# stelleg/caster-dta

Hardware: AMD Instinct MI355X
Metric: graph-pairs/sec (Davis-shaped protein+drug), encoders fwd+bwd (higher is better)
Workload: dtype f32; 1 GPU; davis_b64; pairs_per_gpu=64, residues_per_gpu=19200, protein_edges_per_gpu=57484, atoms_per_gpu=2560, drug_edges_per_gpu=7986, encoder=CASTER-DTA(2,2), pass=fwdbwd, activation_storage=fp32, scope=encoders, torch_compile=False, tunable_gemms=False, two_lane_head=False, train_mode=True, csr_build_in_step=True, hip_graph=True, kernels=mfma

## Files before the change

caster-dta_amd/csrc/gvp_quad.h:

```cpp
#pragma once
#include <hip/hip_runtime.h>

#include "gvp_math.h"

namespace gq {

typedef float f4 __attribute__((ext_vector_type(4)));

constexpr int P1 = 0, P2 = 1;
constexpr int ceil4(int x) { return (x + 3) / 4; }

struct bf16s {};
template <typename ST> struct Io;
template <> struct Io<float> {
  static constexpr bool BF = false;
  static __device__ __forceinline__ f4 ld4(const float* p, int64_t i) { return *reinterpret_cast<const f4*>(p + i); }
  static __device__ __forceinline__ float ld(const float* p, int64_t i) { return p[i]; }
  static __device__ __forceinline__ void st4(float* p, int64_t i, f4 v) { *reinterpret_cast<f4*>(p + i) = v; }
  static __device__ __forceinline__ void st(float* p, int64_t i, float v) { p[i] = v; }
  static __device__ __forceinline__ float rt(float v) { return v; }
  static __device__ __forceinline__ f4 rt4(f4 v) { return v; }
};
struct f32_gvpdef {};
struct f32_linear {};
template <> struct Io<bf16s> {
  static constexpr bool BF = true;
  static __device__ __forceinline__ float widen(uint32_t hi16) { return __uint_as_float(hi16); }
  static __device__ __forceinline__ uint16_t narrow(float v) { return __builtin_bit_cast(uint16_t, (__bf16)v); }
  static __device__ __forceinline__ f4 ld4(const float* p, int64_t i) {
    const uint2 u = *reinterpret_cast<const uint2*>(reinterpret_cast<const uint16_t*>(p) + i);
    return f4{widen(u.x << 16), widen(u.x & 0xffff0000u), widen(u.y << 16), widen(u.y & 0xffff0000u)};
  }
  static __device__ __forceinline__ float ld(const float* p, int64_t i) {
    return widen((uint32_t)reinterpret_cast<const uint16_t*>(p)[i] << 16);
  }
  static __device__ __forceinline__ void st4(float* p, int64_t i, f4 v) {
    uint2 u;
    u.x = (uint32_t)narrow(v[0]) | ((uint32_t)narrow(v[1]) << 16);
    u.y = (uint32_t)narrow(v[2]) | ((uint32_t)narrow(v[3]) << 16);
    *reinterpret_cast<uint2*>(reinterpret_cast<uint16_t*>(p) + i) = u;
  }
  static __device__ __forceinline__ void st(float* p, int64_t i, float v) { reinterpret_cast<uint16_t*>(p)[i] = narrow(v); }
  static __device__ __forceinline__ float rt(float v) { return widen((uint32_t)narrow(v) << 16); }
  static __device__ __forceinline__ f4 rt4(f4 v) { return f4{rt(v[0]), rt(v[1]), rt(v[2]), rt(v[3])}; }
};

template <> struct Io<f32_gvpdef> : Io<float> {};
template <> struct Io<f32_linear> : Io<float> {};

template <int KIND, int BASE, int WIDTH>
struct Seg {
  static_assert(KIND == P2 || WIDTH % 16 == 0, "P1 segments are whole 16-channel tiles");
  static constexpr int steps = KIND == P1 ? WIDTH / 4 : ceil4(WIDTH);
  static __host__ __device__ int col(int s, int g) {
    if (KIND == P1) return BASE + 16 * (s >> 2) + 4 * g + (s & 3);
    const int c = 4 * s + g;
    return c < WIDTH ? BASE + c : -1;
  }
};

template <int STEPS>
struct SegNone {
  static constexpr int steps = STEPS;
  static __host__ __device__ int col(int, int) { return -1; }
};

template <class... S>
struct Segs {
  static constexpr int steps = (S::steps + ... + 0);
  static __host__ __device__ int col(int s, int g) {
    int res = -1, s0 = 0;
    ((res = (s >= s0 && s < s0 + S::steps) ? S::col(s - s0, g) : res, s0 += S::steps), ...);
    return res;
  }
};

template <int NSTEPS>
__host__ __device__ inline void frag_decode(int idx, int& mt, int& s, int& lane) {
  constexpr int REGION = NSTEPS * 64, FULL = NSTEPS / 4;
  mt = idx / REGION;
  const int u = idx - mt * REGION;
  if (u < FULL * 256) { s = 4 * (u >> 8) + (u & 3); lane = (u & 255) >> 2; }
  else { const int v = u - FULL * 256; s = 4 * FULL + (v >> 6); lane = v & 63; }
}
// ... 917 lines not shown
          for (int j = 0; j < TN; ++j) outer_items<1, 1, BF>(AV[j], BH[j], w.vv);
        }
      }
    }
    if constexpr (PACK_V) {
#pragma unroll
      for (int p = 0; p < 3; ++p) {
        f4 A2[TN][1], B2[TN][1];
#pragma unroll
        for (int j = 0; j < TN; ++j) {
          float a2[VOR + HR], b2[HR + VSTEPS];
#pragma unroll
          for (int r = 0; r < VOR; ++r) a2[r] = gr[j].dvp[p][r];
#pragma unroll
          for (int r = 0; r < HR; ++r) a2[VOR + r] = gr[j].dvh[p][r];
#pragma unroll
          for (int r = 0; r < HR; ++r) b2[r] = c[j].vh[p][r];
#pragma unroll
          for (int s_ = 0; s_ < VSTEPS; ++s_) b2[HR + s_] = bv[j][p][s_];
          transpose_slots<VOR + HR>(a2, A2[j], lane, tscr + j * TSCR_FLOATS);
          transpose_slots<HR + VSTEPS>(b2, B2[j], lane, tscr + j * TSCR_FLOATS);
        }
#pragma unroll
        for (int j = 0; j < TN; ++j) outer_items<1, 1, BF>(A2[j], B2[j], w.vv);
      }
    } else {
#pragma unroll
      for (int p = 0; p < 3; ++p) {
        f4 AH[TN][1], BI[TN][1];
#pragma unroll
        for (int j = 0; j < TN; ++j) {
          float ah[HR], bin[VSTEPS];
#pragma unroll
          for (int r = 0; r < HR; ++r) ah[r] = gr[j].dvh[p][r];
#pragma unroll
          for (int s = 0; s < VSTEPS; ++s) bin[s] = bv[j][p][s];
          transpose_slots<HR>(ah, AH[j], lane, tscr + j * TSCR_FLOATS);
          transpose_slots<VSTEPS>(bin, BI[j], lane, tscr + j * TSCR_FLOATS);
        }
#pragma unroll
        for (int j = 0; j < TN; ++j) outer_items<1, 1, BF>(AH[j], BI[j], w.vh_);
      }
    }
  }
  template <class Acc>
  static __device__ __forceinline__ void wacc_flush(const WAcc& w, float* gblk, int lane) {
    const int i = lane & 15, g = lane >> 4;
    const bool first = false;
    flush_slots<Acc, Segs<Seg<P1, 0, SO>>, WsCols, OT, NBT>(gblk + A::ws(NT), first, K, w.ws, lane);
#pragma unroll
    for (int t = 0; t < OT; ++t) {
      float tot[4];
      float* q[4];
      bool on[4];
#pragma unroll
      for (int r = 0; r < 4; ++r) {
        tot[r] = row_total(w.bs[t][r]);
        q[r] = gblk + A::bs(NT) + 16 * t + 4 * g + r;
        on[r] = i == 15;
      }
      add_where<Acc, 4>(q, on, tot);
    }
    if (VO > 0) {
      flush_slots<Acc, Segs<Seg<P2, 0, (VO > 0 ? VO : 1)>>, Segs<Seg<P1, 0, SO>>, 1, OT>(gblk + A::wsv(NT), first, SO, w.wsv, lane);
      float tot[VOR];
      float* q[VOR];
      bool on[VOR];
#pragma unroll
      for (int r = 0; r < VOR; ++r) {
        tot[r] = row_total(w.bsv[r]);
        q[r] = gblk + A::bsv(NT) + 4 * r + g;
        on[r] = i == 15 && 4 * r + g < VO;
      }
      add_where<Acc, VOR>(q, on, tot);
      if constexpr (!PACK_V)
        flush_slots<Acc, Segs<Seg<P2, 0, (VO > 0 ? VO : 1)>>, Segs<Seg<P2, 0, H>>, 1, 1>(gblk + A::wv(NT), first, H, w.vv, lane);
    }
    if constexpr (PACK_V) {
      flush_slots<Acc, Segs<Seg<P2, 0, (VO > 0 ? VO : 1)>, SegNone<HR>>, Segs<Seg<P2, 0, H>, SegNone<VSTEPS>>, 1, 1>(
          gblk + A::wv(NT), first, H, w.vv, lane);
      flush_slots<Acc, Segs<SegNone<VOR>, Seg<P2, 0, H>>, Segs<SegNone<HR>, VSegs>, 1, 1>(gblk, first, VI, w.vv, lane);
    } else {
      flush_slots<Acc, Segs<Seg<P2, 0, H>>, VSegs, 1, 1>(gblk, first, VI, w.vh_, lane);
    }
  }
};

template <int S, int NV>
__device__ __forceinline__ void ln_quad(const float* ln, int lane, f4 (&s)[S / 16], float (&v)[3][ceil4(NV)]) {
  const int g = lane >> 4;
  float sum = 0.f;
#pragma unroll
  for (int t = 0; t < S / 16; ++t) sum += s[t][0] + s[t][1] + s[t][2] + s[t][3];
  const float mean = quad_sum(sum) * (1.0f / S);
  float var = 0.f;
#pragma unroll
  for (int t = 0; t < S / 16; ++t)
#pragma unroll
    for (int r = 0; r < 4; ++r) { const float d = s[t][r] - mean; var = fmaf(d, d, var); }
  const float rstd = gvp::f_rsqrt(quad_sum(var) * (1.0f / S) + gvp::kLnEps);
#pragma unroll
  for (int t = 0; t < S / 16; ++t) {
    const f4 ga = *reinterpret_cast<const f4*>(ln + 16 * t + 4 * g);
    const f4 be = *reinterpret_cast<const f4*>(ln + S + 16 * t + 4 * g);
#pragma unroll
    for (int r = 0; r < 4; ++r) s[t][r] = fmaf((s[t][r] - mean) * rstd, ga[r], be[r]);
  }
  float n2 = 0.f;
#pragma unroll
  for (int r = 0; r < ceil4(NV); ++r)
    if (4 * r + g < NV)
      n2 += gvp::f_max(v[0][r] * v[0][r] + v[1][r] * v[1][r] + v[2][r] * v[2][r], gvp::kNormEps);
  const float rvn = gvp::f_rsqrt(quad_sum(n2) * (1.0f / NV));
#pragma unroll
  for (int p = 0; p < 3; ++p)
#pragma unroll
    for (int r = 0; r < ceil4(NV); ++r) v[p][r] *= rvn;
}

template <int S, int NV>
__device__ __forceinline__ void ln_quad_bwd(const float* ln, int lane, const f4 (&x)[S / 16],
                                            const float (&v)[3][ceil4(NV)], f4 (&ds)[S / 16],
                                            float (&dv)[3][ceil4(NV)], f4 (&dgamma)[S / 16], f4 (&dbeta)[S / 16]) {
  const int g = lane >> 4;
  float sum = 0.f;
#pragma unroll
  for (int t = 0; t < S / 16; ++t) sum += x[t][0] + x[t][1] + x[t][2] + x[t][3];
  const float mean = quad_sum(sum) * (1.0f / S);
  float var = 0.f;
#pragma unroll
  for (int t = 0; t < S / 16; ++t)
#pragma unroll
    for (int r = 0; r < 4; ++r) { const float d = x[t][r] - mean; var = fmaf(d, d, var); }
  const float rstd = gvp::f_rsqrt(quad_sum(var) * (1.0f / S) + gvp::kLnEps);
  f4 xh[S / 16], dxh[S / 16];
  float m1 = 0.f, m2 = 0.f;
#pragma unroll
  for (int t = 0; t < S / 16; ++t) {
    const f4 ga = *reinterpret_cast<const f4*>(ln + 16 * t + 4 * g);
#pragma unroll
    for (int r = 0; r < 4; ++r) {
      xh[t][r] = (x[t][r] - mean) * rstd;
      dgamma[t][r] = ds[t][r] * xh[t][r];
      dbeta[t][r] = ds[t][r];
      dxh[t][r] = ds[t][r] * ga[r];
      m1 += dxh[t][r];
      m2 = fmaf(dxh[t][r], xh[t][r], m2);
    }
  }
  m1 = quad_sum(m1) * (1.0f / S);
  m2 = quad_sum(m2) * (1.0f / S);
#pragma unroll
  for (int t = 0; t < S / 16; ++t)
#pragma unroll
    for (int r = 0; r < 4; ++r) ds[t][r] = rstd * (dxh[t][r] - m1 - xh[t][r] * m2);
  float n2s = 0.f, dot = 0.f;
  bool free_[ceil4(NV)];
#pragma unroll
  for (int r = 0; r < ceil4(NV); ++r) {
    free_[r] = false;
    if (4 * r + g < NV) {
      const float n2 = v[0][r] * v[0][r] + v[1][r] * v[1][r] + v[2][r] * v[2][r];
      free_[r] = n2 > gvp::kNormEps;
      n2s += gvp::f_max(n2, gvp::kNormEps);
      dot += dv[0][r] * v[0][r] + dv[1][r] * v[1][r] + dv[2][r] * v[2][r];
    }
// ... 65 lines not shown
```

caster-dta_amd/csrc/gvp_quad_bwd_kernels.hip:

```cpp
#include <hip/hip_runtime.h>
#include <stdint.h>
#include <stdlib.h>

#include <type_traits>

#include "gvp_internal.h"
#include "gvp_quad.h"

using namespace gq;

#ifdef CGVP_STAMPS
__device__ unsigned long long* g_stamp_buf_bwd = nullptr;
extern "C" int cgvp_debug_set_stamp_buffer_bwd(unsigned long long* buf) {
  return (int)hipMemcpyToSymbol(HIP_SYMBOL(g_stamp_buf_bwd), &buf, sizeof(buf));
}
#endif

namespace {

constexpr int WAVE = 64;
constexpr int TILE = 16;

#ifdef CGVP_STAMPS
#define STAMP(slot)                                                                          \
// ... 28 lines not shown
__device__ __forceinline__ int opaque_lane(int lane) {
  asm volatile("" : "+v"(lane));
  return lane;
}

template <int BLK>
__device__ __forceinline__ void zero_block(float* gblk, int lane) {
  static_assert(BLK % 4 == 0, "blocks are whole float4s");
  for (int k = lane; k < BLK / 4; k += WAVE) reinterpret_cast<f4*>(gblk)[k] = f4{0.f, 0.f, 0.f, 0.f};
}
template <int BLK, int PW, int WPB_ = 8>
__device__ __forceinline__ void write_slab_row(float* slab, const float* blocks, int row = blockIdx.x) {
  __syncthreads();
  float* out = slab + (size_t)row * BLK;
  for (int k = threadIdx.x; k < BLK; k += WAVE * WPB_) {
    float t = 0.f;
#pragma unroll
    for (int ww = 0; ww < WPB_; ++ww) t += blocks[ww * PW + k];
    out[k] = t;
  }
}

template <int NFLOATS, int NTHR>
__device__ __forceinline__ void stage_slice(float* lds, const float* __restrict__ src, int tid) {
  static_assert(NFLOATS % 4 == 0, "image slices are whole float4s");
  constexpr int NF4 = NFLOATS / 4, IT = (NF4 + NTHR - 1) / NTHR;
  const f4* s = reinterpret_cast<const f4*>(src);
  f4* d = reinterpret_cast<f4*>(lds);
  f4 v[IT];
#pragma unroll
  for (int k = 0; k < IT; ++k) { const int idx = tid + k * NTHR; if (idx < NF4) v[k] = s[idx]; }
#pragma unroll
  for (int k = 0; k < IT; ++k) { const int idx = tid + k * NTHR; if (idx < NF4) d[idx] = v[k]; }
}

constexpr int cmax(int a, int b) { return a > b ? a : b; }
template <bool ONE> using AccFor = typename std::conditional<ONE, AccStoreOnce, AccPriv>::type;
constexpr int pad4(int x) { return (x + 3) / 4 * 4; }

template <class Acc, int S>
__device__ __forceinline__ void ln_param_grads(float* blk, bool first, int lane, bool active,
                                               const f4 (&dgamma)[S / 16], const f4 (&dbeta)[S / 16]) {
  const int i = lane & 15, g = lane >> 4;
#pragma unroll
  for (int t = 0; t < S / 16; ++t) {
    float tot[8];
    float* q[8];
    bool on[8];
#pragma unroll
    for (int r = 0; r < 4; ++r) {
      tot[r] = row_total(active ? dgamma[t][r] : 0.f);
      tot[4 + r] = row_total(active ? dbeta[t][r] : 0.f);
      q[r] = blk + 16 * t + 4 * g + r;
      q[4 + r] = blk + S + 16 * t + 4 * g + r;
      on[r] = on[4 + r] = i == 15;
    }
    add_where<Acc, 8>(q, on, tot);
  }
}

constexpr int NB_LN0 = 0, NB_LN1 = 2 * NS, NB_FF0 = 4 * NS, NB_FF1 = NB_FF0 + LFf0::size(0),
              NODE_BLK = NB_FF1 + LFf1::size(0);
constexpr int HB_LN = 0, HB_GVP = 2 * NS, HEAD_BLK = HB_GVP + LHead::size(0);
constexpr int NODE_GB = pad4(NODE_BLK), HEAD_GB = pad4(HEAD_BLK);

constexpr int MROW = NS + NV;
__device__ __forceinline__ void node_dropout(const float* mask, const gvp::RngArgs& rng, int which, int64_t n, int g,
                                             f4& ms, float& mv) {
  if (mask) {
    ms = *reinterpret_cast<const f4*>(mask + n * MROW + 4 * g);
    mv = mask[n * MROW + NS + g];
  } else if (rng.seed) {
    const unsigned long long seed = rng.seed[0], off = rng.seed[1];
    float fs[4];
    gvp::dropout_row20(seed, off, rng.stream + which, n, g, rng.p, fs, mv);
    ms = f4{fs[0], fs[1], fs[2], fs[3]};
  }
}
struct NodeBArgs {
  const float* img_node; const float* imgT_node;
  const float* h; const float* dh; const float* mask0; const float* mask1; gvp::RngArgs rng;
  const float* g_up0; const float* g_up1; const float* g_up2;
  int64_t N; float* g_dh; float* g_h; float* zero_rows; float* slab;
};
constexpr int node_bwd_lds_floats() { return BW_TPB + Image<0, 0>::ND_SIZE + Image<0, 0>::TN_SIZE + BW_WPB * (NODE_GB + TSCR_FLOATS); }
static_assert(node_bwd_lds_floats() * 4 <= 160 * 1024, "node backward LDS plan exceeds the CU");

template <typename ST, bool ONE = false>
__device__ __forceinline__ void node_bwd_body(const NodeBArgs& a, float* lds) {
  typedef Image<0, 0> IM;
  typedef AccFor<ONE> Acc;
  float* f_node = lds + BW_TPB;
  float* t_node = f_node + IM::ND_SIZE;
  float* blocks = t_node + IM::TN_SIZE;
  const int lane0 = threadIdx.x & 63, w = threadIdx.x >> 6;
  float* gblk = blocks + w * NODE_GB;
  float* tscr = blocks + BW_WPB * NODE_GB + w * TSCR_FLOATS;
  stage_slice<IM::ND_SIZE, BW_TPB>(f_node, a.img_node, threadIdx.x);
  stage_slice<IM::TN_SIZE, BW_TPB>(t_node, a.imgT_node, threadIdx.x);
  zero_block<NODE_GB>(gblk, lane0);
  STAMP(0);
  __syncthreads();
  STAMP(1);

  const f4 zero = {0.f, 0.f, 0.f, 0.f};
  const int zt[1] = {0};
  const bool first = false;
  const int64_t ntiles = (a.N + TILE - 1) / TILE;
  for (int64_t tile = (int64_t)w * gridDim.x + blockIdx.x; tile < ntiles; tile += (int64_t)gridDim.x * BW_WPB) {
    const int lane = opaque_lane(lane0), i = lane & 15, g = lane >> 4;
    const int64_t n = tile * TILE + i;
    const bool active = n < a.N;
    f4 x0[1] = {zero};
    float xv0[3][1] = {{0.f}, {0.f}, {0.f}};
    f4 m0s = {1.f, 1.f, 1.f, 1.f}, m1s = {1.f, 1.f, 1.f, 1.f};
    float m0v = 1.f, m1v = 1.f;
    f4 gs[1] = {zero};
    float gv[3][1] = {{0.f}, {0.f}, {0.f}};
    if (active) {
      const int64_t hr = n * ROW;
      node_dropout(a.mask0, a.rng, 0, n, g, m0s, m0v);
      node_dropout(a.mask1, a.rng, 1, n, g, m1s, m1v);
      x0[0] = Io<ST>::ld4(a.h, hr + 4 * g) + Io<ST>::ld4(a.dh, hr + 4 * g) * m0s;
#pragma unroll
      for (int p = 0; p < 3; ++p) xv0[p][0] = Io<ST>::ld(a.h, hr + NS + 3 * g + p) + Io<ST>::ld(a.dh, hr + NS + 3 * g + p) * m0v;
      const float* ups[3] = {a.g_up0, a.g_up1, a.g_up2};
#pragma unroll
      for (int u = 0; u < 3; ++u)
        if (ups[u]) {
          const float* r_ = ups[u] + n * ROW;
          gs[0] += *reinterpret_cast<const f4*>(r_ + 4 * g);
#pragma unroll
          for (int p = 0; p < 3; ++p) gv[p][0] += r_[NS + 3 * g + p];
        }
    }
    f4 y[1] = {x0[0]};
    float yv[3][1] = {{xv0[0][0]}, {xv0[1][0]}, {xv0[2][0]}};
    ln_quad<NS, NV>(f_node + IM::ND_LN0, lane, y, yv);
    f4 hs[1][4], s2[1][1];
    float hv[1][3][2], v2[1][3][1];
    float bs0[1][4], bv0[1][3][1], bs1[1][16], bv1[1][3][2];
    typename Ff0<ST>::Cache c0[1];
    typename Ff1<ST>::Cache c1[1];
#pragma unroll
    for (int r = 0; r < 4; ++r) bs0[0][r] = y[0][r];
#pragma unroll
    for (int p = 0; p < 3; ++p) bv0[0][p][0] = yv[p][0];
    Ff0<ST>::template forward<1, Io<ST>::BF>(f_node + IM::ND_FF0, lane, zt, bs0, bv0, hs, hv, c0);
#pragma unroll
    for (int t = 0; t < 4; ++t)
#pragma unroll
      for (int r = 0; r < 4; ++r) bs1[0][4 * t + r] = hs[0][t][r];
#pragma unroll
    for (int p = 0; p < 3; ++p) { bv1[0][p][0] = hv[0][p][0]; bv1[0][p][1] = hv[0][p][1]; }
    Ff1<ST>::template forward<1, Io<ST>::BF>(f_node + IM::ND_FF1, lane, zt, bs1, bv1, s2, v2, c1);
    f4 z[1] = {y[0] + s2[0][0] * m1s};
    float zv[3][1];
#pragma unroll
    for (int p = 0; p < 3; ++p) zv[p][0] = yv[p][0] + v2[0][p][0] * m1v;

    STAMP(2);
    STAMP(3);
    {
      f4 dga[1], dbe[1];
      ln_quad_bwd<NS, NV>(f_node + IM::ND_LN1, lane, z, zv, gs, gv, dga, dbe);
      ln_param_grads<Acc, NS>(gblk + NB_LN1, first, lane, active, dga, dbe);
    }
    float d_hs[16], d_hv[3][2];
    {
      f4 d_so[1] = {gs[0] * m1s};
      float d_vo[3][1] = {{gv[0][0] * m1v}, {gv[1][0] * m1v}, {gv[2][0] * m1v}};
      typename Ff1<ST>::Grads gr1;
      STAMP(4);
      Ff1<ST>::template backward<Io<ST>::BF>(t_node + IM::TN_FF1, lane, c1[0], d_so, d_vo, d_hs, d_hv, gr1);
      STAMP(5);
      Ff1<ST>::template weight_grads<Acc, Io<ST>::BF>(gblk + NB_FF1, first, lane, 0, active, bs1[0], bv1[0], c1[0], gr1, tscr);
    }
    {
      f4 d_so[4];
#pragma unroll
      for (int t = 0; t < 4; ++t) d_so[t] = f4{d_hs[4 * t], d_hs[4 * t + 1], d_hs[4 * t + 2], d_hs[4 * t + 3]};
      float d_ys[4], d_yv[3][1];
      typename Ff0<ST>::Grads gr0;
      STAMP(6);
      Ff0<ST>::template backward<Io<ST>::BF>(t_node + IM::TN_FF0, lane, c0[0], d_so, d_hv, d_ys, d_yv, gr0);
      STAMP(7);
      Ff0<ST>::template weight_grads<Acc, Io<ST>::BF>(gblk + NB_FF0, first, lane, 0, active, bs0[0], bv0[0], c0[0], gr0, tscr);
#pragma unroll
      for (int r = 0; r < 4; ++r) gs[0][r] += d_ys[r];
#pragma unroll
      for (int p = 0; p < 3; ++p) gv[p][0] += d_yv[p][0];
    }
    STAMP(8);
    {
      f4 dga[1], dbe[1];
      ln_quad_bwd<NS, NV>(f_node + IM::ND_LN0, lane, x0, xv0, gs, gv, dga, dbe);
      ln_param_grads<Acc, NS>(gblk + NB_LN0, first, lane, active, dga, dbe);
    }
    if (active) {
      if (a.g_h) {
        float* row = a.g_h + n * ROW;
        *reinterpret_cast<f4*>(row + 4 * g) = gs[0];
#pragma unroll
        for (int p = 0; p < 3; ++p) row[NS + 3 * g + p] = gv[p][0];
      }
      float* row = a.g_dh + n * ROW;
      *reinterpret_cast<f4*>(row + 4 * g) = gs[0] * m0s;
#pragma unroll
      for (int p = 0; p < 3; ++p) row[NS + 3 * g + p] = gv[p][0] * m0v;
      if (a.zero_rows) {
        float* z = a.zero_rows + n * ROW;
        *reinterpret_cast<f4*>(z + 4 * g) = zero;
#pragma unroll
        for (int p = 0; p < 3; ++p) z[NS + 3 * g + p] = 0.f;
      }
    }
  }
  STAMP(9);
  write_slab_row<NODE_GB, NODE_GB>(a.slab, blocks);
  STAMP(10);
}
template <typename ST, bool ONE = false>
__global__ __launch_bounds__(BW_TPB, 2) void node_bwd_kernel(NodeBArgs a) {
  WALL_STAMP(0);
  extern __shared__ __attribute__((aligned(16))) float lds[];
  node_bwd_body<ST, ONE>(a, lds);
}

struct HeadBArgs {
  const float* img_head; const float* imgT_head; const float* h_out; const float* g_out;
  int64_t N; float* g_h_out; float* slab;
};
constexpr int head_bwd_lds_floats() { return BW_TPB + Image<0, 0>::HD_SIZE + Image<0, 0>::TH_SIZE + BW_WPB * (HEAD_GB + TSCR_FLOATS); }

template <typename ST, bool ONE = false>
__device__ __forceinline__ void head_bwd_body(const HeadBArgs& a, float* lds) {
  typedef Image<0, 0> IM;
  typedef AccFor<ONE> Acc;
  float* f_head = lds + BW_TPB;
  float* t_head = f_head + IM::HD_SIZE;
  float* blocks = t_head + IM::TH_SIZE;
  const int lane = threadIdx.x & 63, w = threadIdx.x >> 6;
  float* gblk = blocks + w * HEAD_GB;
  float* tscr = blocks + BW_WPB * HEAD_GB + w * TSCR_FLOATS;
  stage_slice<IM::HD_SIZE, BW_TPB>(f_head, a.img_head, threadIdx.x);
  stage_slice<IM::TH_SIZE, BW_TPB>(t_head, a.imgT_head, threadIdx.x);
  zero_block<HEAD_GB>(gblk, lane);
  __syncthreads();

  const int i = lane & 15, g = lane >> 4;
  const f4 zero = {0.f, 0.f, 0.f, 0.f};
  const int zt[1] = {0};
  const bool first = false;
  const int64_t ntiles = (a.N + TILE - 1) / TILE;
  for (int64_t tile = (int64_t)w * gridDim.x + blockIdx.x; tile < ntiles; tile += (int64_t)gridDim.x * BW_WPB) {
    const int64_t n = tile * TILE + i;
    const bool active = n < a.N;
    f4 o1[1] = {zero};
    float ov1[3][1] = {{0.f}, {0.f}, {0.f}};
    f4 d_o[4] = {zero, zero, zero, zero};
    if (active) {
      const int64_t hr = n * ROW;
      o1[0] = Io<ST>::ld4(a.h_out, hr + 4 * g);
#pragma unroll
      for (int p = 0; p < 3; ++p) ov1[p][0] = Io<ST>::ld(a.h_out, hr + NS + 3 * g + p);
      const float* gr_ = a.g_out + n * OUT;
#pragma unroll
      for (int t = 0; t < 4; ++t) d_o[t] = *reinterpret_cast<const f4*>(gr_ + 16 * t + 4 * g);
    }
    f4 wsn[1] = {o1[0]};
    float wvn[3][1] = {{ov1[0][0]}, {ov1[1][0]}, {ov1[2][0]}};
    ln_quad<NS, NV>(f_head + IM::HD_LN, lane, wsn, wvn);
    float bsh[1][4], bvh[1][3][1], dummy[1][3][1];
#pragma unroll
    for (int r = 0; r < 4; ++r) bsh[0][r] = wsn[0][r];
#pragma unroll
    for (int p = 0; p < 3; ++p) bvh[0][p][0] = wvn[p][0];
    f4 o[1][4];
    QHead::Cache ch[1];
    QHead::template forward<1, Io<ST>::BF>(f_head + IM::HD_GVP, lane, zt, bsh, bvh, o, dummy, ch);
    float d_vo[3][1] = {{0.f}, {0.f}, {0.f}}, d_bs[4], d_bv[3][1];
    QHead::Grads grh;
    QHead::template backward<Io<ST>::BF>(t_head, lane, ch[0], d_o, d_vo, d_bs, d_bv, grh);
    QHead::template weight_grads<Acc, Io<ST>::BF>(gblk + HB_GVP, first, lane, 0, active, bsh[0], bvh[0], ch[0], grh, tscr);
    f4 dws[1] = {f4{d_bs[0], d_bs[1], d_bs[2], d_bs[3]}};
    float dwv[3][1] = {{d_bv[0][0]}, {d_bv[1][0]}, {d_bv[2][0]}};
    f4 dga[1], dbe[1];
    ln_quad_bwd<NS, NV>(f_head + IM::HD_LN, lane, o1, ov1, dws, dwv, dga, dbe);
    ln_param_grads<Acc, NS>(gblk + HB_LN, first, lane, active, dga, dbe);
    if (active) {
      float* row = a.g_h_out + n * ROW;
      *reinterpret_cast<f4*>(row + 4 * g) = dws[0];
#pragma unroll
      for (int p = 0; p < 3; ++p) row[NS + 3 * g + p] = dwv[p][0];
    }
  }
  write_slab_row<HEAD_GB, HEAD_GB>(a.slab, blocks);
}
template <typename ST>
__global__ __launch_bounds__(BW_TPB, 2) void head_bwd_kernel(HeadBArgs a) {
  WALL_STAMP(1);
  extern __shared__ __attribute__((aligned(16))) float lds[];
  head_bwd_body<ST>(a, lds);
}

template <typename ST, bool ONE = false>
__global__ __launch_bounds__(BW_TPB, 2) void node_head_bwd_kernel(HeadBArgs hd, NodeBArgs a) {
  WALL_STAMP(0);
  extern __shared__ __attribute__((aligned(16))) float lds[];
  head_bwd_body<ST, ONE>(hd, lds);
  __syncthreads();
  node_bwd_body<ST, ONE>(a, lds);
}

constexpr int EROW = quad::kEdgeRow;
template <int NTE>
struct ConvBlk {
  static constexpr int M0 = 0, M1 = M0 + LMsg0::size(0), M2 = M1 + LMsg::size(0), SIZE = pad4(M2 + LMsg::size(0));
};
#ifndef CGVP_CONV_BWD_WAVES
#define CGVP_CONV_BWD_WAVES 8
#endif
constexpr int CB_WPB = CGVP_CONV_BWD_WAVES, CB_TPB = WAVE * CB_WPB, CB_MAX_GRID = BW_MAX_GRID;
constexpr int CB_SCR = TSCR_FLOATS;
static_assert(CB_SCR >= (TILE / 2) * ROW + TILE, "g_src transpose fits the scratch");
template <int NTE>
struct ConvBImg {
  typedef Image<0, NTE> IM;
  static constexpr int F0 = IM::CV_M0, FSIZE = IM::CV_SIZE - IM::CV_M0;
  static constexpr int T0 = IM::TC_M0, TSIZE = IM::TC_SIZE - IM::TC_M0;
};
template <int NTE>
constexpr int conv_bwd_lds_floats() { return CB_TPB + ConvBImg<NTE>::FSIZE + ConvBImg<NTE>::TSIZE + CB_WPB * (ConvBlk<NTE>::SIZE + CB_SCR); }
static_assert(conv_bwd_lds_floats<1>() * 4 <= 160 * 1024 && conv_bwd_lds_floats<0>() * 4 <= 160 * 1024, "conv backward LDS plan exceeds the CU");

struct ConvBArgs {
  const float* img; const float* imgT;
  const float* h; const float* e_emb;
  const int32_t* rowptr; const int32_t* esrc; const int32_t* edst;
  int64_t N; int npw; int mean; const float* g_dh; float* g_src; float* g_dst; float* g_e; float* slab;
  float* g_edge; float* slot;
};

template <int NTE, typename ST>
__global__ __launch_bounds__(CB_TPB, CB_WPB / 4) void conv_bwd_kernel(ConvBArgs a) {
  WALL_STAMP(2);
  typedef Image<0, NTE> IM;
  typedef ConvBImg<NTE> BI;
  typedef ConvBlk<NTE> B;
  constexpr int PW = B::SIZE + CB_SCR;
  extern __shared__ __attribute__((aligned(16))) float lds[];
  float* img = lds + CB_TPB - BI::F0;
  float* imgT = lds + CB_TPB + BI::FSIZE - BI::T0;
  const int lane0 = threadIdx.x & 63, w = threadIdx.x >> 6;
  float* blocks = lds + CB_TPB + BI::FSIZE + BI::TSIZE;
  float* gblk = blocks + w * PW;
  float* scr = gblk + B::SIZE;
#ifdef CGVP_MFMA_TRANSPOSE
  float* const CB_TSCR = nullptr;
#else
  float* const CB_TSCR = scr;
#endif
  stage_slice<BI::FSIZE, CB_TPB>(lds + CB_TPB, a.img + BI::F0, threadIdx.x);
  stage_slice<BI::TSIZE, CB_TPB>(lds + CB_TPB + BI::FSIZE, a.imgT + BI::T0, threadIdx.x);
  for (int k = lane0; k < B::SIZE / 4; k += WAVE) reinterpret_cast<f4*>(gblk)[k] = f4{0.f, 0.f, 0.f, 0.f};
  STAMP(0);
  __syncthreads();
  STAMP(1);

  const f4 zero = {0.f, 0.f, 0.f, 0.f};
  const int zt[1] = {0};
  const int64_t ngroups = (a.N + a.npw - 1) / a.npw;
  const int64_t grp0 = (int64_t)blockIdx.x * CB_WPB + w;
  const bool first = false;
  float carry[7] = {0.f, 0.f, 0.f, 0.f, 0.f, 0.f, 0.f};
  int carry_dst = -1;
  for (int64_t grp = grp0; grp < ngroups; grp += (int64_t)gridDim.x * CB_WPB) {
    const int64_t n0 = grp * a.npw;
    const int nn = (int)((a.N - n0 < a.npw) ? (a.N - n0) : a.npw);
    const int32_t e0 = a.rowptr[n0], e1 = a.rowptr[n0 + nn];
    for (int k = lane0; k < nn * ROW; k += WAVE) {
      const int64_t nd = n0 + k / ROW;
      if (a.rowptr[nd + 1] == a.rowptr[nd]) a.g_dst[n0 * ROW + k] = 0.f;
    }
    for (int32_t base = e0; base < e1; base += TILE) {
      const int lane = opaque_lane(lane0), i = lane & 15, g = lane >> 4;
      const int32_t p = base + i;
      const bool active = p < e1;
      f4 es0 = zero, es1 = zero, sj = zero, si = zero, d_ms = zero;
      float ev[3] = {0.f, 0.f, 0.f}, vj[3] = {0.f, 0.f, 0.f}, vi[3] = {0.f, 0.f, 0.f}, d_mv[3] = {0.f, 0.f, 0.f};
      int32_t src = 0, dst = -1;
      if (active) {
        src = a.esrc[p];
        dst = a.edst[p];
        const int64_t er = (int64_t)p * EROW;
// ... 737 lines not shown
struct SegTable { cgvp_segment s[CGVP_MAX_SEGS]; };
template <bool ADD = true>
__global__ __launch_bounds__(RED_COLS * RED_RG) void reduce_segments_kernel(SegTable t, float* __restrict__ grad, int overwrite) {
  __shared__ float part[RED_RG][RED_COLS];
  const cgvp_segment sg = t.s[blockIdx.y];
  const int c = threadIdx.x & (RED_COLS - 1), rg = threadIdx.x / RED_COLS;
  const int j = blockIdx.x * RED_COLS + c;
  if (blockIdx.x * RED_COLS >= sg.len) return;
  float s = 0.f;
  if (j < sg.len) {
    const float* col = sg.slab + sg.col0 + j;
    float s0 = 0.f, s1 = 0.f, s2 = 0.f, s3 = 0.f;
    int r = rg;
    for (; r + 3 * RED_RG < sg.rows; r += 4 * RED_RG) {
      s0 += col[(size_t)r * sg.stride];
      s1 += col[(size_t)(r + RED_RG) * sg.stride];
      s2 += col[(size_t)(r + 2 * RED_RG) * sg.stride];
      s3 += col[(size_t)(r + 3 * RED_RG) * sg.stride];
    }
    for (; r < sg.rows; r += RED_RG) s0 += col[(size_t)r * sg.stride];
    s = (s0 + s1) + (s2 + s3);
  }
  part[rg][c] = s;
  __syncthreads();
  if (rg == 0 && j < sg.len) {
    float tt = 0.f;
#pragma unroll
    for (int k = 0; k < RED_RG; ++k) tt += part[k][c];
    if (!ADD || overwrite) grad[sg.dst + j] = tt;
    else atomicAdd(grad + sg.dst + j, tt);
  }
}

template <bool ADD = true>
__global__ __launch_bounds__(256) void reduce_segments_rows_kernel(SegTable t, float* __restrict__ grad, int overwrite) {
  const cgvp_segment sg = t.s[blockIdx.y];
  const int j = blockIdx.x * 256 + threadIdx.x;
  if (j >= sg.len) return;
  const float* col = sg.slab + sg.col0 + j;
  float s = 0.f;
  for (int r = 0; r < sg.rows; ++r) s += col[(size_t)r * sg.stride];
  if (!ADD || overwrite) grad[sg.dst + j] = s;
  else atomicAdd(grad + sg.dst + j, s);
}

struct SrcSumArgs {
  const float* rows; const float* self; const int32_t* sptr; const int32_t* spos;
  const int32_t* rowptr; const float* slot; int64_t waves; int64_t N; float* out;
};
template <int W>
__global__ __launch_bounds__(256) void src_sum_kernel(SrcSumArgs a) {
  const int64_t t = (int64_t)blockIdx.x * 256 + threadIdx.x;
  if (t >= a.N * W) return;
  const int64_t n = t / W;
  const int c = (int)(t - n * W);
  float s = a.self ? a.self[t] : 0.f;
  const int32_t k0 = a.sptr[n], k1 = a.sptr[n + 1];
#pragma unroll 4
  for (int32_t k = k0; k < k1; ++k) s += a.rows[(int64_t)a.spos[k] * W + c];
  if (a.slot) {
    const int64_t ev = a.rowptr[a.N];
    const int64_t iters = (ev + TILE - 1) / TILE, chunk = (iters + a.waves - 1) / a.waves * TILE;
    const int64_t r0 = a.rowptr[n], r1 = a.rowptr[n + 1];
    if (chunk > 0)
      for (int64_t w = r0 / chunk + 1; w * chunk < r1; ++w) s += a.slot[w * W + c];
  }
  a.out[t] = s;
}

inline int bwd_grid_cap(int64_t units) {
  static const int forced = [] {
    const char* e = getenv("CGVP_BWD_GRID");
    const int v = e ? atoi(e) : 0;
    return (v >= 1 && v <= BW_MAX_GRID) ? v : 0;
  }();
  if (forced) return forced;
  constexpr int SMALL = BW_MAX_GRID - 8;
  return units <= (int64_t)SMALL * BW_WPB ? SMALL : BW_MAX_GRID;
}
inline bool one_tile_per_wave(int64_t tiles, int grid) {
  static const bool on = [] { const char* e = getenv("CGVP_BWD_STORE_ONCE"); return !(e && e[0] == '0'); }();
  return on && tiles <= (int64_t)grid * BW_WPB;
}
inline int grid_for(int64_t tiles) {
  const int cap = bwd_grid_cap(tiles);
  return (int)(tiles < 1 ? 1 : (tiles > cap ? cap : tiles));
}

}

namespace quad {

int bwd_block_sizes(int nt_node, int nt_edge, BwdBlocks* b) {
  if (nt_node == 0) b->emb = EmbBlk<0>::SIZE; else if (nt_node == 20) b->emb = EmbBlk<20>::SIZE;
  else if (nt_node == 21) b->emb = EmbBlk<21>::SIZE; else return CGVP_ERR_UNSUPPORTED_DIMS;
  if (nt_edge == 0) { b->conv_edge = EdgeBlk<0>::SIZE; b->conv_total = ConvBlk<0>::SIZE; }
  else if (nt_edge == 1) { b->conv_edge = EdgeBlk<1>::SIZE; b->conv_total = ConvBlk<1>::SIZE; }
  else return CGVP_ERR_UNSUPPORTED_DIMS;
  b->node = NODE_GB;
  b->head = HEAD_GB;
  return 0;
}

template <bool ADD>
void launch_reduce_segments(const SegTable& t, int nsegs, int maxlen, int maxrows, float* grad_params, hipStream_t st,
                            int overwrite) {
  if (maxrows <= 32) {
    launch<reduce_segments_rows_kernel<ADD>>(dim3((maxlen + 255) / 256, nsegs), dim3(256), 0, st, t, grad_params, overwrite);
    return;
  }
  launch<reduce_segments_kernel<ADD>>(dim3((maxlen + RED_COLS - 1) / RED_COLS, nsegs), dim3(RED_COLS * RED_RG), 0,
                                      st, t, grad_params, overwrite);
}

int reduce_segments(const cgvp_segment* segs, int nsegs, float* grad_params, hipStream_t st, int overwrite, bool store_only) {
  if (nsegs <= 0) return 0;
  SegTable t;
  int maxlen = 0;
  int maxrows = 0;
  for (int i = 0; i < nsegs; ++i) {
    t.s[i] = segs[i];
    maxlen = segs[i].len > maxlen ? segs[i].len : maxlen;
    maxrows = segs[i].rows > maxrows ? segs[i].rows : maxrows;
  }
  if (store_only) launch_reduce_segments<false>(t, nsegs, maxlen, maxrows, grad_params, st, 1);
  else launch_reduce_segments<true>(t, nsegs, maxlen, maxrows, grad_params, st, overwrite);
  return 0;
}

int src_sum(int width, const float* rows, const float* self, const int32_t* sptr, const int32_t* spos,
            const int32_t* rowptr, const float* slot, int64_t waves, int64_t N, float* out, hipStream_t st) {
  if (N <= 0) return 0;
  SrcSumArgs a{rows, self, sptr, spos, rowptr, slot, waves, N, out};
  const unsigned blocks = (unsigned)((N * width + 255) / 256);
  switch (width) {
    case 16: return launch<src_sum_kernel<16>>(dim3(blocks), dim3(256), 0, st, a);
    case ROW: return launch<src_sum_kernel<ROW>>(dim3(blocks), dim3(256), 0, st, a);
    case 41: return launch<src_sum_kernel<41>>(dim3(blocks), dim3(256), 0, st, a);
    case 52: return launch<src_sum_kernel<52>>(dim3(blocks), dim3(256), 0, st, a);
    default: return CGVP_ERR_UNSUPPORTED_DIMS;
  }
}

int conv_bwd_max_waves() { return BW_MAX_GRID * 8; }

int reduce_slab(const float* slab, int rows, int stride, int col0, int len, float* dst, hipStream_t st) {
  if (rows <= 32) {
    launch<reduce_rows_kernel>(dim3((len + 255) / 256), dim3(256), 0, st, slab, rows, stride, col0, len, dst);
    return 0;
  }
  launch<reduce_slab_kernel>(dim3((len + RED_COLS - 1) / RED_COLS), dim3(RED_COLS * RED_RG), 0, st, slab, rows, stride, col0, len, dst);
  return 0;
}

int node_update_bwd(const float* img_node, const float* imgT_node, const float* h, const float* dh,
                    const float* mask0, const float* mask1, gvp::RngArgs rng, const float* g_up0, const float* g_up1,
                    const float* g_up2, int64_t N, float* g_dh, float* g_h, float* zero_rows, float* slab, int* grid,
                    int policy, hipStream_t st) {
  NodeBArgs a{img_node, imgT_node, h, dh, mask0, mask1, rng, g_up0, g_up1, g_up2, N, g_dh, g_h, zero_rows, slab};
  const int64_t tiles = (N + TILE - 1) / TILE;
  const int G = grid_for(tiles);
  *grid = G;
  const size_t lds = (size_t)node_bwd_lds_floats() * sizeof(float);
  return with_policy<true>(policy, [&](auto tag) {
    using ST = typename decltype(tag)::type;
    return with_flag(one_tile_per_wave(tiles, G), [&](auto one) {
      return launch<node_bwd_kernel<ST, one.value>>(dim3(G), dim3(BW_TPB), lds, st, a);
    });
  });
}

int node_head_bwd(const float* img_head, const float* imgT_head, const float* h_out, const float* g_out, float* g_h_out,
                  float* head_slab, const float* img_node, const float* imgT_node, const float* h, const float* dh,
                  const float* mask0, const float* mask1, gvp::RngArgs rng, int64_t N, float* g_dh, float* g_h,
                  float* zero_rows, float* slab, int* grid, int policy, hipStream_t st) {
  HeadBArgs hd{img_head, imgT_head, h_out, g_out, N, g_h_out, head_slab};
  NodeBArgs a{img_node, imgT_node, h, dh, mask0, mask1, rng, g_h_out, nullptr, nullptr, N, g_dh, g_h, zero_rows, slab};
  const int64_t tiles = (N + TILE - 1) / TILE;
  const int G = grid_for(tiles);
  *grid = G;
  const int f = node_bwd_lds_floats() > head_bwd_lds_floats() ? node_bwd_lds_floats() : head_bwd_lds_floats();
  const size_t lds = (size_t)f * sizeof(float);
  return with_policy<false>(policy, [&](auto tag) {
    using ST = typename decltype(tag)::type;
    return with_flag(one_tile_per_wave(tiles, G), [&](auto one) {
      return launch<node_head_bwd_kernel<ST, one.value>>(dim3(G), dim3(BW_TPB), lds, st, hd, a);
    });
  });
}

int head_bwd(const float* img_head, const float* imgT_head, const float* h_out, const float* g_out, int64_t N,
             float* g_h_out, float* slab, int* grid, int policy, hipStream_t st) {
  HeadBArgs a{img_head, imgT_head, h_out, g_out, N, g_h_out, slab};
  const int G = grid_for((N + TILE - 1) / TILE);
  *grid = G;
  const size_t lds = (size_t)head_bwd_lds_floats() * sizeof(float);
  return with_policy<false>(policy, [&](auto tag) {
    return launch<head_bwd_kernel<typename decltype(tag)::type>>(dim3(G), dim3(BW_TPB), lds, st, a);
  });
}

int conv_bwd_version() {
  static const int v = [] {
    const char* e = getenv("CGVP_CONV_BWD");
    return (e && e[0] == '1') ? 1 : ((e && e[0] == '2') ? 2 : 3);
  }();
  return v;
}

template <int NTE, int TN, int WPB_, bool STORE>
int conv_bwd2_impl(ConvBArgs& a, int64_t E, int* grid, int policy, hipStream_t st) {
  typedef C2Shape<TN, WPB_> SH;
  const int64_t iters = (E + TN * TILE - 1) / (TN * TILE);
  const int64_t wgs = (iters + WPB_ - 1) / WPB_;
  const int cap = bwd_grid_cap(((E + TILE - 1) / TILE + 1) / 2);
  const int G = (int)(wgs < 1 ? 1 : (wgs > cap ? cap : wgs));
  *grid = G;
  const size_t lds = (size_t)SH::template lds_floats<NTE>() * sizeof(float);
  return with_policy<NTE == 0>(policy, [&](auto tag) {
    return launch<conv_bwd2_kernel<NTE, typename decltype(tag)::type, TN, WPB_, STORE>>(dim3(G), dim3(SH::TPB), lds, st, a);
  });
}

template <int NTE>
int conv_bwd_impl(ConvBArgs& a, int* grid, int policy, hipStream_t st) {
  const int64_t ngroups = (a.N + a.npw - 1) / a.npw;
  const int64_t wgs = (ngroups + CB_WPB - 1) / CB_WPB;
  const int cap = bwd_grid_cap(ngroups);
  const int G = (int)(wgs < 1 ? 1 : (wgs > cap ? cap : wgs));
  *grid = G;
  const size_t lds = (size_t)conv_bwd_lds_floats<NTE>() * sizeof(float);
  return with_policy<NTE == 0>(policy, [&](auto tag) {
    return launch<conv_bwd_kernel<NTE, typename decltype(tag)::type>>(dim3(G), dim3(CB_TPB), lds, st, a);
  });
}

template <int NTE>
int conv_bwd_version_impl(ConvBArgs& a, int64_t E, int* grid, int policy, hipStream_t st) {
  if (a.g_edge) return conv_bwd2_impl<NTE, 1, 8, true>(a, E, grid, policy, st);
  if (conv_bwd_version() == 2) return conv_bwd2_impl<NTE, 2, 4, false>(a, E, grid, policy, st);
  if (conv_bwd_version() == 3) return conv_bwd2_impl<NTE, 1, 8, false>(a, E, grid, policy, st);
  return conv_bwd_impl<NTE>(a, grid, policy, st);
}

int conv_bwd(int nt_edge, const float* img, const float* imgT, const float* h, const float* e_emb,
             const int32_t* rowptr, const int32_t* esrc, const int32_t* edst, int64_t N, int64_t E, int mean,
             const float* g_dh, float* g_src, float* g_dst, float* g_e, float* slab, int* grid, int policy, hipStream_t st,
             float* g_edge, float* slot) {
  int64_t deg = N > 0 ? (E + N - 1) / N : 1;
  if (deg < 1) deg = 1;
  int npw = (int)((2 * TILE - 2) / deg);
  npw = npw < 1 ? 1 : (npw > WAVE ? WAVE : npw);
  ConvBArgs a{img, imgT, h, e_emb, rowptr, esrc, edst, N, npw, mean, g_dh, g_src, g_dst, g_e, slab, g_edge, slot};
  if (g_edge && (conv_bwd_version() != 3 || !slot)) return CGVP_ERR_NONDETERMINISTIC;
  if (nt_edge == 0) return conv_bwd_version_impl<0>(a, E, grid, policy, st);
  if (nt_edge == 1) return conv_bwd_version_impl<1>(a, E, grid, policy, st);
  return CGVP_ERR_UNSUPPORTED_DIMS;
}

template <int NTE>
int edge_bwd_impl(EdgeBArgs& a, int* grid, int policy, hipStream_t st) {
  const int64_t tiles = (a.E + TILE - 1) / TILE;
  const int G = (int)(tiles < 1 ? 1 : (tiles > 2 * bwd_grid_cap((tiles + 1) / 2) ? 2 * bwd_grid_cap((tiles + 1) / 2) : tiles));
  *grid = G;
  const size_t lds = (size_t)edge_bwd_lds_floats<NTE>() * sizeof(float);
  return with_policy<false>(policy, [&](auto tag) {
    using ST = typename decltype(tag)::type;
    return with_flag(a.g_e_s != nullptr, [&](auto dx) {
      return launch<edge_bwd_kernel<NTE, ST, dx.value>>(dim3(G), dim3(BW_TPB), lds, st, a);
// ... 42 lines not shown
```

Before: 280,200 graph-pairs/sec.

## Add cooperative block-level weight-gradient reduction to node backward kernel

In the one-tile-per-wave fp32 node backward path, each wave now writes its weight-gradient operands to swizzled LDS tiles instead of accumulating per-wave weight gradients. After a barrier, the waves split the output blocks and reduce across wave slots with MFMA, writing one slab row per block. FF0 operands are kept in registers and emitted after FF1's reduction so the two can share LDS, and LayerNorm parameter partials are staged and summed the same way. The aim is to cut redundant per-wave accumulation and flush work, at the cost of more registers, extra barriers and more LDS use. The path is on by default only for the kernel without the head; the fused head kernel needs an environment flag set to 2.

```diff
diff --git a/caster-dta_amd/csrc/gvp_quad.h b/caster-dta_amd/csrc/gvp_quad.h
--- a/caster-dta_amd/csrc/gvp_quad.h
+++ b/caster-dta_amd/csrc/gvp_quad.h
@@ -1,5 +1,7 @@
 #pragma once
 #include <hip/hip_runtime.h>
+
+#include <type_traits>
 
 #include "gvp_math.h"
 
@@ -1083,6 +1085,164 @@
       flush_slots<Acc, Segs<SegNone<VOR>, Seg<P2, 0, H>>, Segs<SegNone<HR>, VSegs>, 1, 1>(gblk, first, VI, w.vv, lane);
     } else {
       flush_slots<Acc, Segs<Seg<P2, 0, H>>, VSegs, 1, 1>(gblk, first, VI, w.vh_, lane);
+    }
+  }
+
+  static constexpr int OP_TILE = 256;
+  static constexpr int OPS_AWS = 0, OPS_BWS = OPS_AWS + OT, OPS_AWSV = OPS_BWS + NBT, OPS_BWSV = OPS_AWSV + 1,
+                       OPS_AV = OPS_BWSV + OT, OPS_BV = OPS_AV + 3, OPS_TILES = OPS_BV + 3;
+  static constexpr int OPS_FLOATS = OPS_TILES * OP_TILE;
+  static constexpr int WG_BLOCKS = OT * NBT + OT + 1;
+  typedef typename std::conditional<(NT > 0), WsCols, Segs<SegNone<1>, SSegs, Seg<P2, NT + SI, H>>>::type CoopWsCols;
+
+  struct Kept {
+    float bs[SSTEPS], bv[3][VSTEPS];
+    Cache c;
+    Grads gr;
+    bool active;
+  };
+  static __device__ __forceinline__ void keep(Kept& k, bool active, const float (&bs)[SSTEPS], const float (&bv)[3][VSTEPS],
+                                              const Cache& c, const Grads& gr) {
+    k.active = active;
+#pragma unroll
+    for (int s = 0; s < SSTEPS; ++s) k.bs[s] = bs[s];
+#pragma unroll
+    for (int p = 0; p < 3; ++p) {
+#pragma unroll
+      for (int s = 0; s < VSTEPS; ++s) k.bv[p][s] = bv[p][s];
+      k.c.vh[p] = c.vh[p];
+      k.gr.dvp[p] = gr.dvp[p];
+      k.gr.dvh[p] = gr.dvh[p];
+    }
+#pragma unroll
+    for (int r = 0; r < HR; ++r) k.c.vn[r] = c.vn[r];
+#pragma unroll
+    for (int t = 0; t < OT; ++t) { k.c.sp[t] = c.sp[t]; k.gr.dsp[t] = gr.dsp[t]; }
+    k.gr.dgate = gr.dgate;
+  }
+  template <int N>
+  static __device__ __forceinline__ void put_slots(float* tiles, const float (&v)[N], int lane) {
+    const int i = lane & 15, g = lane >> 4;
+#pragma unroll
+    for (int s = 0; s < N; ++s) {
+      const int r = s & 3;
+      tiles[(s >> 2) * OP_TILE + (4 * r + g) * 16 + 4 * ((i >> 2) ^ r) + (i & 3)] = v[s];
+    }
+  }
+  static __device__ __forceinline__ f4 get_slots(const float* tile, int lane) {
+    const int n = lane & 15, gq_ = lane >> 4;
+    return *reinterpret_cast<const f4*>(tile + n * 16 + 4 * (gq_ ^ (n >> 2)));
+  }
+  static __device__ __forceinline__ void emit_operands(float* ops, int lane, int type, bool active,
+                                                       const float (&bs)[SSTEPS], const float (&bv)[3][VSTEPS],
+                                                       const Cache& c, const Grads& gr) {
+    static_assert(PACK_V, "the cooperative path is written for GVPs whose dWv and dWh share a block");
+    const int g = lane >> 4;
+    {
+      float a[4 * OT], b[NBW];
+#pragma unroll
+      for (int t = 0; t < OT; ++t)
+#pragma unroll
+        for (int r = 0; r < 4; ++r) a[4 * t + r] = active ? gr.dsp[t][r] : 0.f;
+#pragma unroll
+      for (int s = 0; s < (NT > 0 ? NTS : 1); ++s) b[s] = (NT > 0 && 4 * s + g == type) ? 1.f : 0.f;
+#pragma unroll
+      for (int s = 0; s < SSTEPS; ++s) b[(NT > 0 ? NTS : 1) + s] = bs[s];
+#pragma unroll
+      for (int r = 0; r < HR; ++r) b[(NT > 0 ? NTS : 1) + SSTEPS + r] = c.vn[r];
+      put_slots(ops + OPS_AWS * OP_TILE, a, lane);
+      put_slots(ops + OPS_BWS * OP_TILE, b, lane);
+    }
+    {
+      float a[VOR], b[4 * OT];
+#pragma unroll
+      for (int r = 0; r < VOR; ++r) a[r] = active ? gr.dgate[r] : 0.f;
+#pragma unroll
+      for (int t = 0; t < OT; ++t)
+#pragma unroll
+        for (int r = 0; r < 4; ++r) b[4 * t + r] = c.sp[t][r];
+      put_slots(ops + OPS_AWSV * OP_TILE, a, lane);
+      put_slots(ops + OPS_BWSV * OP_TILE, b, lane);
+    }
+#pragma unroll
+    for (int p = 0; p < 3; ++p) {
+      float a2[VOR + HR], b2[HR + VSTEPS];
+#pragma unroll
+      for (int r = 0; r < VOR; ++r) a2[r] = active ? gr.dvp[p][r] : 0.f;
+#pragma unroll
+      for (int r = 0; r < HR; ++r) a2[VOR + r] = active ? gr.dvh[p][r] : 0.f;
+#pragma unroll
+      for (int r = 0; r < HR; ++r) b2[r] = c.vh[p][r];
+#pragma unroll
+      for (int s_ = 0; s_ < VSTEPS; ++s_) b2[HR + s_] = bv[p][s_];
+      put_slots(ops + (OPS_AV + p) * OP_TILE, a2, lane);
+      put_slots(ops + (OPS_BV + p) * OP_TILE, b2, lane);
+    }
+  }
+  template <class RowSegs, class ColSegs>
+  static __device__ __forceinline__ void store_block(float* dst, int LD, int mt, int nt, const f4& acc, int lane) {
+    const int n = lane & 15, gq_ = lane >> 4;
+    const int cs = 4 * nt + (n >> 2), rs = 4 * mt + gq_;
+    const int col = cs < ColSegs::steps ? ColSegs::col(cs, n & 3) : -1;
+#pragma unroll
+    for (int r = 0; r < 4; ++r) {
+      const int row = rs < RowSegs::steps ? RowSegs::col(rs, r) : -1;
+      if (row >= 0 && col >= 0) dst[row * LD + col] = acc[r];
+    }
+  }
+  template <int B>
+  static __device__ __forceinline__ void reduce_block(const float* ops, int stride, int nslots, float* gout, int lane) {
+    const int n = lane & 15, gq_ = lane >> 4;
+    f4 acc = {0.f, 0.f, 0.f, 0.f};
+    if constexpr (B < OT * NBT) {
+      constexpr int X = B / NBT, Y = B % NBT;
+      float tot = 0.f;
+      for (int s = 0; s < nslots; ++s) {
+        const f4 a = get_slots(ops + s * stride + (OPS_AWS + X) * OP_TILE, lane);
+        const f4 b = get_slots(ops + s * stride + (OPS_BWS + Y) * OP_TILE, lane);
+#pragma unroll
+        for (int rr = 0; rr < 4; ++rr) acc = mfma(a[rr], b[rr], acc);
+        if (Y == 0) tot += (a[0] + a[1]) + (a[2] + a[3]);
+      }
+      store_block<Segs<Seg<P1, 0, SO>>, CoopWsCols>(gout + A::ws(NT), K, X, Y, acc, lane);
+      if (Y == 0) {
+        tot = quad_sum(tot);
+        if (gq_ == 0) gout[A::bs(NT) + Seg<P1, 0, SO>::col(4 * X + (n >> 2), n & 3)] = tot;
+      }
+    } else if constexpr (B < OT * NBT + OT) {
+      constexpr int Y = B - OT * NBT;
+      float tot = 0.f;
+      for (int s = 0; s < nslots; ++s) {
+        const f4 a = get_slots(ops + s * stride + OPS_AWSV * OP_TILE, lane);
+        const f4 b = get_slots(ops + s * stride + (OPS_BWSV + Y) * OP_TILE, lane);
+#pragma unroll
+        for (int rr = 0; rr < 4; ++rr) acc = mfma(a[rr], b[rr], acc);
+        if (Y == 0) tot += (a[0] + a[1]) + (a[2] + a[3]);
+      }
+      store_block<Segs<Seg<P2, 0, (VO > 0 ? VO : 1)>>, Segs<Seg<P1, 0, SO>>>(gout + A::wsv(NT), SO, 0, Y, acc, lane);
+      if (Y == 0) {
+        tot = quad_sum(tot);
+        if (gq_ == 0 && n < VO) gout[A::bsv(NT) + n] = tot;
+      }
+    } else {
+      for (int s = 0; s < nslots; ++s)
+#pragma unroll
+        for (int p = 0; p < 3; ++p) {
+          const f4 a = get_slots(ops + s * stride + (OPS_AV + p) * OP_TILE, lane);
+          const f4 b = get_slots(ops + s * stride + (OPS_BV + p) * OP_TILE, lane);
+#pragma unroll
+          for (int rr = 0; rr < 4; ++rr) acc = mfma(a[rr], b[rr], acc);
+        }
+      store_block<Segs<Seg<P2, 0, (VO > 0 ? VO : 1)>, SegNone<HR>>, Segs<Seg<P2, 0, H>, SegNone<VSTEPS>>>(gout + A::wv(NT), H, 0, 0,
+                                                                                                         acc, lane);
+      store_block<Segs<SegNone<VOR>, Seg<P2, 0, H>>, Segs<SegNone<HR>, VSegs>>(gout, VI, 0, 0, acc, lane);
+    }
+  }
+  template <int NW, int B = 0>
+  static __device__ __forceinline__ void reduce_blocks(const float* ops, int stride, int nslots, float* gout, int lane, int w) {
+    if constexpr (B < WG_BLOCKS) {
+      if (w == B % NW) reduce_block<B>(ops, stride, nslots, gout, lane);
+      reduce_blocks<NW, B + 1>(ops, stride, nslots, gout, lane, w);
     }
   }
 };
diff --git a/caster-dta_amd/csrc/gvp_quad_bwd_kernels.hip b/caster-dta_amd/csrc/gvp_quad_bwd_kernels.hip
--- a/caster-dta_amd/csrc/gvp_quad_bwd_kernels.hip
+++ b/caster-dta_amd/csrc/gvp_quad_bwd_kernels.hip
@@ -134,12 +134,38 @@
   const float* h; const float* dh; const float* mask0; const float* mask1; gvp::RngArgs rng;
   const float* g_up0; const float* g_up1; const float* g_up2;
   int64_t N; float* g_dh; float* g_h; float* zero_rows; float* slab;
+  int coop = 0;
 };
 constexpr int node_bwd_lds_floats() { return BW_TPB + Image<0, 0>::ND_SIZE + Image<0, 0>::TN_SIZE + BW_WPB * (NODE_GB + TSCR_FLOATS); }
 static_assert(node_bwd_lds_floats() * 4 <= 160 * 1024, "node backward LDS plan exceeds the CU");
 
-template <typename ST, bool ONE = false>
+struct NodeCoopLds {
+  static constexpr int IMG = BW_TPB, OPS1 = IMG + Image<0, 0>::ND_SIZE + Image<0, 0>::TN_SIZE,
+                       LNP = OPS1 + BW_WPB * QFf1::OPS_FLOATS, END1 = LNP + BW_WPB * 4 * NS,
+                       OPS0 = BW_TPB, END0 = OPS0 + BW_WPB * QFf0::OPS_FLOATS;
+};
+static_assert(NodeCoopLds::END1 <= node_bwd_lds_floats() && NodeCoopLds::END0 <= node_bwd_lds_floats(),
+              "cooperative node backward LDS plan exceeds the launch's allocation");
+static_assert(NodeCoopLds::OPS1 % 4 == 0 && NB_LN1 == NB_LN0 + 2 * NS, "store alignment / norm.0 | norm.1 are adjacent");
+
+template <int S>
+__device__ __forceinline__ void ln_param_partials(float* part, int lane, bool active, const f4 (&dgamma)[S / 16],
+                                                  const f4 (&dbeta)[S / 16]) {
+  const int i = lane & 15, g = lane >> 4;
+  float* const trash = AccPriv::trash();
+#pragma unroll
+  for (int t = 0; t < S / 16; ++t)
+#pragma unroll
+    for (int r = 0; r < 4; ++r) {
+      const float tg = row_total(active ? dgamma[t][r] : 0.f), tb = row_total(active ? dbeta[t][r] : 0.f);
+      *(i == 15 ? part + 16 * t + 4 * g + r : trash) = tg;
+      *(i == 15 ? part + S + 16 * t + 4 * g + r : trash) = tb;
+    }
+}
+
+template <typename ST, bool ONE = false, bool COOP = false>
 __device__ __forceinline__ void node_bwd_body(const NodeBArgs& a, float* lds) {
+  static_assert(!COOP || (ONE && !Io<ST>::BF), "the cooperative path is the fp32 single-tile case");
   typedef Image<0, 0> IM;
   typedef AccFor<ONE> Acc;
   float* f_node = lds + BW_TPB;
@@ -150,7 +176,11 @@
   float* tscr = blocks + BW_WPB * NODE_GB + w * TSCR_FLOATS;
   stage_slice<IM::ND_SIZE, BW_TPB>(f_node, a.img_node, threadIdx.x);
   stage_slice<IM::TN_SIZE, BW_TPB>(t_node, a.imgT_node, threadIdx.x);
-  zero_block<NODE_GB>(gblk, lane0);
+  const bool coop = COOP && a.coop;
+  if (!coop) zero_block<NODE_GB>(gblk, lane0);
+  float* ops1 = lds + NodeCoopLds::OPS1 + w * Ff1<ST>::OPS_FLOATS;
+  float* lnp = lds + NodeCoopLds::LNP + w * 4 * NS;
+  typename Ff0<ST>::Kept keep0;
   STAMP(0);
   __syncthreads();
   STAMP(1);
@@ -216,7 +246,8 @@
     {
       f4 dga[1], dbe[1];
       ln_quad_bwd<NS, NV>(f_node + IM::ND_LN1, lane, z, zv, gs, gv, dga, dbe);
-      ln_param_grads<Acc, NS>(gblk + NB_LN1, first, lane, active, dga, dbe);
+      if (coop) ln_param_partials<NS>(lnp + 2 * NS, lane, active, dga, dbe);
+      else ln_param_grads<Acc, NS>(gblk + NB_LN1, first, lane, active, dga, dbe);
     }
     float d_hs[16], d_hv[3][2];
     {
@@ -226,7 +257,8 @@
       STAMP(4);
       Ff1<ST>::template backward<Io<ST>::BF>(t_node + IM::TN_FF1, lane, c1[0], d_so, d_vo, d_hs, d_hv, gr1);
       STAMP(5);
-      Ff1<ST>::template weight_grads<Acc, Io<ST>::BF>(gblk + NB_FF1, first, lane, 0, active, bs1[0], bv1[0], c1[0], gr1, tscr);
+      if (coop) Ff1<ST>::emit_operands(ops1, lane, 0, active, bs1[0], bv1[0], c1[0], gr1);
+      else Ff1<ST>::template weight_grads<Acc, Io<ST>::BF>(gblk + NB_FF1, first, lane, 0, active, bs1[0], bv1[0], c1[0], gr1, tscr);
     }
     {
       f4 d_so[4];
@@ -237,7 +269,11 @@
       STAMP(6);
       Ff0<ST>::template backward<Io<ST>::BF>(t_node + IM::TN_FF0, lane, c0[0], d_so, d_hv, d_ys, d_yv, gr0);
       STAMP(7);
-      Ff0<ST>::template weight_grads<Acc, Io<ST>::BF>(gblk + NB_FF0, first, lane, 0, active, bs0[0], bv0[0], c0[0], gr0, tscr);
+      if (coop) {
+        Ff0<ST>::keep(keep0, active, bs0[0], bv0[0], c0[0], gr0);
+      } else {
+        Ff0<ST>::template weight_grads<Acc, Io<ST>::BF>(gblk + NB_FF0, first, lane, 0, active, bs0[0], bv0[0], c0[0], gr0, tscr);
+      }
 #pragma unroll
       for (int r = 0; r < 4; ++r) gs[0][r] += d_ys[r];
 #pragma unroll
@@ -247,7 +283,8 @@
     {
       f4 dga[1], dbe[1];
       ln_quad_bwd<NS, NV>(f_node + IM::ND_LN0, lane, x0, xv0, gs, gv, dga, dbe);
-      ln_param_grads<Acc, NS>(gblk + NB_LN0, first, lane, active, dga, dbe);
+      if (coop) ln_param_partials<NS>(lnp, lane, active, dga, dbe);
+      else ln_param_grads<Acc, NS>(gblk + NB_LN0, first, lane, active, dga, dbe);
     }
     if (active) {
       if (a.g_h) {
@@ -267,16 +304,39 @@
         for (int p = 0; p < 3; ++p) z[NS + 3 * g + p] = 0.f;
       }
     }
+    if constexpr (COOP) break;
   }
   STAMP(9);
-  write_slab_row<NODE_GB, NODE_GB>(a.slab, blocks);
+  if (coop) {
+    int nslots = 0;
+#pragma unroll
+    for (int ww = 0; ww < BW_WPB; ++ww) nslots += (int64_t)ww * gridDim.x + blockIdx.x < ntiles ? 1 : 0;
+    float* row = a.slab + (size_t)blockIdx.x * NODE_GB;
+    __syncthreads();
+    Ff1<ST>::template reduce_blocks<BW_WPB>(lds + NodeCoopLds::OPS1, Ff1<ST>::OPS_FLOATS, nslots, row + NB_FF1, lane0, w);
+    if (threadIdx.x < 4 * NS) {
+      float t = 0.f;
+      for (int s = 0; s < nslots; ++s) t += lds[NodeCoopLds::LNP + s * 4 * NS + threadIdx.x];
+      row[NB_LN0 + threadIdx.x] = t;
+    } else if (threadIdx.x - 4 * NS < NODE_GB - NODE_BLK) {
+      row[NODE_BLK + threadIdx.x - 4 * NS] = 0.f;
+    }
+    __syncthreads();
+    if (w < nslots)
+      Ff0<ST>::emit_operands(lds + NodeCoopLds::OPS0 + w * Ff0<ST>::OPS_FLOATS, lane0, 0, keep0.active, keep0.bs, keep0.bv,
+                             keep0.c, keep0.gr);
+    __syncthreads();
+    Ff0<ST>::template reduce_blocks<BW_WPB>(lds + NodeCoopLds::OPS0, Ff0<ST>::OPS_FLOATS, nslots, row + NB_FF0, lane0, w);
+  } else {
+    write_slab_row<NODE_GB, NODE_GB>(a.slab, blocks);
+  }
   STAMP(10);
 }
-template <typename ST, bool ONE = false>
+template <typename ST, bool ONE = false, bool COOP = false>
 __global__ __launch_bounds__(BW_TPB, 2) void node_bwd_kernel(NodeBArgs a) {
   WALL_STAMP(0);
   extern __shared__ __attribute__((aligned(16))) float lds[];
-  node_bwd_body<ST, ONE>(a, lds);
+  node_bwd_body<ST, ONE, COOP>(a, lds);
 }
 
 struct HeadBArgs {
@@ -356,13 +416,13 @@
   head_bwd_body<ST>(a, lds);
 }
 
-template <typename ST, bool ONE = false>
+template <typename ST, bool ONE = false, bool COOP = false>
 __global__ __launch_bounds__(BW_TPB, 2) void node_head_bwd_kernel(HeadBArgs hd, NodeBArgs a) {
   WALL_STAMP(0);
   extern __shared__ __attribute__((aligned(16))) float lds[];
   head_bwd_body<ST, ONE>(hd, lds);
   __syncthreads();
-  node_bwd_body<ST, ONE>(a, lds);
+  node_bwd_body<ST, ONE, COOP>(a, lds);
 }
 
 constexpr int EROW = quad::kEdgeRow;
@@ -1266,6 +1326,12 @@
   static const bool on = [] { const char* e = getenv("CGVP_BWD_STORE_ONCE"); return !(e && e[0] == '0'); }();
   return on && tiles <= (int64_t)grid * BW_WPB;
 }
+inline bool coop_wgrad(bool with_head) {
+  if (quad::deterministic_env()) return false;
+  const char* e = getenv("CGVP_BWD_COOP_WGRAD");
+  if (e && e[0] == '0') return false;
+  return !with_head || (e && e[0] == '2');
+}
 inline int grid_for(int64_t tiles) {
   const int cap = bwd_grid_cap(tiles);
   return (int)(tiles < 1 ? 1 : (tiles > cap ? cap : tiles));
@@ -1349,7 +1415,12 @@
   return with_policy<true>(policy, [&](auto tag) {
     using ST = typename decltype(tag)::type;
     return with_flag(one_tile_per_wave(tiles, G), [&](auto one) {
-      return launch<node_bwd_kernel<ST, one.value>>(dim3(G), dim3(BW_TPB), lds, st, a);
+      if constexpr (one.value && std::is_same_v<ST, float>) {
+        a.coop = coop_wgrad(false) ? 1 : 0;
+        return launch<node_bwd_kernel<ST, true, true>>(dim3(G), dim3(BW_TPB), lds, st, a);
+      } else {
+        return launch<node_bwd_kernel<ST, one.value>>(dim3(G), dim3(BW_TPB), lds, st, a);
+      }
     });
   });
 }
@@ -1368,7 +1439,12 @@
   return with_policy<false>(policy, [&](auto tag) {
     using ST = typename decltype(tag)::type;
     return with_flag(one_tile_per_wave(tiles, G), [&](auto one) {
-      return launch<node_head_bwd_kernel<ST, one.value>>(dim3(G), dim3(BW_TPB), lds, st, hd, a);
+      if constexpr (one.value && std::is_same_v<ST, float>) {
+        a.coop = coop_wgrad(true) ? 1 : 0;
+        return launch<node_head_bwd_kernel<ST, true, true>>(dim3(G), dim3(BW_TPB), lds, st, hd, a);
+      } else {
+        return launch<node_head_bwd_kernel<ST, one.value>>(dim3(G), dim3(BW_TPB), lds, st, hd, a);
+      }
     });
   });
 }
```

Result: no change. 280,600 graph-pairs/sec (median of 3 runs) (+0.1%).
